# algbio/GraphChainer

Measured on AMD Instinct MI355X. Metric: reads_per_sec, higher is better.
Workload: dtype u64

## Files before the change

graphchainer_amd/csrc/hip/gc_column_asm.hpp:

```cpp
#pragma once

#define GC_CA_NL "\n\t"
#define GC_CA_SELECT \
	"s_and_b32 m0, s90, 6" GC_CA_NL "s_lshr_b64 s[90:91], s[90:91], 2" GC_CA_NL "s_movrels_b64 %[Eq], s[72:73]" GC_CA_NL
#define GC_CA_COLUMN(M0SET, HN, HP, HNMH, FORCE, STORE) \
	GC_CA_SELECT \
	M0SET GC_CA_NL \
	"s_or_b64 %[Xv], %[Eq], s[82:83]" GC_CA_NL \
	HN \
	"s_and_b64 s[84:85], %[Eq], s[80:81]" GC_CA_NL \
	"s_add_u32 s84, s84, s80" GC_CA_NL \
	"s_addc_u32 s85, s85, s81" GC_CA_NL \
	"s_xor_b64 s[84:85], s[84:85], s[80:81]" GC_CA_NL \
	"s_or_b64 s[84:85], s[84:85], %[Eq]" GC_CA_NL           \
	"s_or_b64 %[Eq], s[84:85], s[80:81]" GC_CA_NL \
	"s_orn2_b64 s[86:87], s[82:83], %[Eq]" GC_CA_NL         \
	"s_and_b64 s[88:89], s[80:81], s[84:85]" GC_CA_NL       \
	"v_writelane_b32 %[plus], s87, m0" GC_CA_NL \
	"v_writelane_b32 %[minus], s89, m0" GC_CA_NL \
	"s_lshl_b64 s[84:85], s[86:87], 1" GC_CA_NL \
	HP                                                      \
	"s_lshl_b64 s[88:89], s[88:89], 1" GC_CA_NL \
	HNMH                                                    \
	"s_or_b64 %[Eq], %[Xv], s[84:85]" GC_CA_NL \
	"s_orn2_b64 s[80:81], s[88:89], %[Eq]" GC_CA_NL         \
	"s_and_b64 s[82:83], s[84:85], %[Xv]" GC_CA_NL          \
	FORCE \
	STORE

#define GC_CA_HN "s_bfe_u64 %[hN], %[pHN], m0" GC_CA_NL "s_or_b64 %[Eq], %[Eq], %[hN]" GC_CA_NL
#define GC_CA_HP "s_bfe_u64 %[Eq], %[pHP], m0" GC_CA_NL "s_or_b64 s[84:85], s[84:85], %[Eq]" GC_CA_NL
#define GC_CA_HP_ONE "s_or_b32 s84, s84, 1" GC_CA_NL
#define GC_CA_HNMH "s_or_b64 s[88:89], s[88:89], %[hN]" GC_CA_NL
#define GC_CA_FORCE "s_bfe_u64 %[hN], %[forced], m0" GC_CA_NL "s_andn2_b64 s[80:81], s[80:81], %[hN]" GC_CA_NL "s_or_b64 s[82:83], s[82:83], %[hN]" GC_CA_NL
#define GC_CA_STORE \
	"v_writelane_b32 %[c0], s80, m0" GC_CA_NL "v_writelane_b32 %[c1], s81, m0" GC_CA_NL "v_writelane_b32 %[c2], s82, m0" GC_CA_NL "v_writelane_b32 %[c3], s83, m0" GC_CA_NL
#define GC_CA_NONE ""

#define GC_CA_LOOP(HN, HP, HNMH, FORCE, STORE) \
	"s_lshr_b64 s[90:91], %[w0], 1" GC_CA_NL \
	"s_min_i32 %[endm1], %[nm1], 0x1001f" GC_CA_NL \
	"s_mov_b32 %[pos], 0x10001\n" \
	"1:" GC_CA_NL                                           \
	"s_cmp_ge_i32 %[pos], %[endm1]" GC_CA_NL \
	"s_cbranch_scc1 3f\n" \
	"2:" GC_CA_NL \
	GC_CA_COLUMN("s_mov_b32 m0, %[pos]", HN, HP, HNMH, FORCE, STORE) \
	GC_CA_COLUMN("s_add_i32 m0, %[pos], 1", HN, HP, HNMH, FORCE, STORE) \
	"s_add_i32 %[pos], %[pos], 2" GC_CA_NL \
	"s_cmp_lt_i32 %[pos], %[endm1]" GC_CA_NL \
	"s_cbranch_scc1 2b\n" \
	"3:" GC_CA_NL                                           \
	"s_cmp_gt_i32 %[pos], %[endm1]" GC_CA_NL \
	"s_cbranch_scc1 4f" GC_CA_NL \
	GC_CA_COLUMN("s_mov_b32 m0, %[pos]", HN, HP, HNMH, FORCE, STORE) \
	"s_add_i32 %[pos], %[pos], 1\n" \
	"4:" GC_CA_NL                                           \
	"s_cmp_ge_i32 %[endm1], %[nm1]" GC_CA_NL \
	"s_cbranch_scc1 6f" GC_CA_NL \
	"s_bitcmp1_b32 %[endm1], 5" GC_CA_NL \
	"s_cbranch_scc1 5f" GC_CA_NL \
	"s_lshl_b64 s[90:91], %[w1], 1" GC_CA_NL \
	"s_min_i32 %[endm1], %[nm1], 0x1003e" GC_CA_NL \
	"s_branch 1b\n" \
	"5:" GC_CA_NL \
	"s_lshr_b64 s[90:91], %[w1], 61" GC_CA_NL \
	"s_mov_b32 %[endm1], %[nm1]" GC_CA_NL \
	"s_branch 1b\n" \
	"6:"

#define GC_CA_OUT_COMMON [VP] "+{s[80:81]}"(VP), [VN] "+{s[82:83]}"(VN), [plus] "+v"(plusWord), [minus] "+v"(minusWord), [Eq] "=&s"(Eq), [Xv] "=&s"(Xv), [pos] "=&s"(pos), [endm1] "=&s"(endm1)
#define GC_CA_OUT_STORE , [c0] "+v"(cr[0]), [c1] "+v"(cr[1]), [c2] "+v"(cr[2]), [c3] "+v"(cr[3])
#define GC_CA_IN_COMMON "{s[72:73]}"(eA), "{s[74:75]}"(eC), "{s[76:77]}"(eG), "{s[78:79]}"(eT), [w0] "s"(w0), [w1] "s"(w1), [nm1] "s"(nm1)
#define GC_CA_CLOBBER "s84", "s85", "s86", "s87", "s88", "s89", "s90", "s91", "m0", "scc"

#if defined(__HIP_DEVICE_COMPILE__)
template <int KIND, int MODE>
__device__ __forceinline__ void gcColumnLoopAsm(uint64_t eA, uint64_t eC, uint64_t eG, uint64_t eT, uint64_t& VP, uint64_t& VN, uint64_t prevHP, uint64_t prevHN, uint64_t forced,
	uint64_t w0, uint64_t w1, int nodeLength, uint32_t& plusWord, uint32_t& minusWord, uint32_t* cr)
{
	const uint32_t nm1 = (uint32_t)__builtin_amdgcn_readfirstlane((nodeLength - 1) | (1 << 16));
	uint64_t Eq, Xv, hN;
	uint32_t pos, endm1;
#pragma clang diagnostic push
#pragma clang diagnostic ignored "-Winline-asm"
	if constexpr (KIND == 2 && MODE == 0)
		asm(GC_CA_LOOP(GC_CA_NONE, GC_CA_HP_ONE, GC_CA_NONE, GC_CA_NONE, GC_CA_NONE)
			: GC_CA_OUT_COMMON : GC_CA_IN_COMMON : GC_CA_CLOBBER);
	else if constexpr (KIND == 2)
		asm(GC_CA_LOOP(GC_CA_NONE, GC_CA_HP_ONE, GC_CA_NONE, GC_CA_NONE, GC_CA_STORE)
			: GC_CA_OUT_COMMON GC_CA_OUT_STORE : GC_CA_IN_COMMON : GC_CA_CLOBBER);
	else if constexpr (KIND == 1 && MODE == 0)
		asm(GC_CA_LOOP(GC_CA_HN, GC_CA_HP, GC_CA_HNMH, GC_CA_NONE, GC_CA_NONE)
			: GC_CA_OUT_COMMON, [hN] "=&s"(hN) : GC_CA_IN_COMMON, [pHP] "s"(prevHP), [pHN] "s"(prevHN) : GC_CA_CLOBBER);
	else if constexpr (KIND == 1)
		asm(GC_CA_LOOP(GC_CA_HN, GC_CA_HP, GC_CA_HNMH, GC_CA_NONE, GC_CA_STORE)
			: GC_CA_OUT_COMMON, [hN] "=&s"(hN) GC_CA_OUT_STORE : GC_CA_IN_COMMON, [pHP] "s"(prevHP), [pHN] "s"(prevHN) : GC_CA_CLOBBER);
	else if constexpr (MODE == 0)
		asm(GC_CA_LOOP(GC_CA_HN, GC_CA_HP, GC_CA_HNMH, GC_CA_FORCE, GC_CA_NONE)
			: GC_CA_OUT_COMMON, [hN] "=&s"(hN) : GC_CA_IN_COMMON, [pHP] "s"(prevHP), [pHN] "s"(prevHN), [forced] "s"(forced) : GC_CA_CLOBBER);
	else
		asm(GC_CA_LOOP(GC_CA_HN, GC_CA_HP, GC_CA_HNMH, GC_CA_FORCE, GC_CA_STORE)
			: GC_CA_OUT_COMMON, [hN] "=&s"(hN) GC_CA_OUT_STORE : GC_CA_IN_COMMON, [pHP] "s"(prevHP), [pHN] "s"(prevHN), [forced] "s"(forced) : GC_CA_CLOBBER);
#pragma clang diagnostic pop
}
#endif
```

graphchainer_amd/csrc/hip/gc_device.hpp:

```cpp
#pragma once
#include <hip/hip_runtime.h>
#include <stdint.h>

#ifndef GC_LOOP_TICK
#define GC_LOOP_TICK(i) ((void)0)
#endif

namespace gcdev {

struct NodeRec {
	uint32_t comp;
	uint32_t outOff;
	uint32_t inOff;
	uint32_t meta;
	uint64_t w0, w1;
};
enum : uint32_t { NODEREC_SLOW = 128u };

struct DGraph {
	uint32_t nNodes;
	uint32_t firstAmbiguous;
	const uint8_t*  nodeLength;
	const uint32_t* nodeOffset;
	const int32_t*  nodeIDs;
// ... 247 lines not shown
{
	uint64_t a = 0, c = 0, g = 0, t = 0;
	int n = len - j;
	if (n > 64) n = 64;
	for (int i = 0; i < n; i++) {
		uint32_t m = iupac[(uint8_t)seq[j + i]];
		uint64_t bit = 1ull << i;
		a |= (m & 1) ? bit : 0ull;
		c |= (m & 2) ? bit : 0ull;
		g |= (m & 4) ? bit : 0ull;
		t |= (m & 8) ? bit : 0ull;
	}
	eq.a = a; eq.c = c; eq.g = g; eq.t = t;
}

struct EqSource {
	const uint64_t* masks;
	uint32_t words;
	uint32_t startBit;
	__device__ __forceinline__ void rows(int len, int j, Eq4& eq) const;
};
__device__ inline void eqVectorBits(const EqSource& src, int len, int j, Eq4& eq)
{
	int n = len - j;
	if (n > 64) n = 64;
	uint32_t bit = src.startBit + (uint32_t)j;
	uint32_t w = bit >> 6, sh = bit & 63;
	uint64_t keep = n >= 64 ? ~0ull : ((1ull << n) - 1);
	uint64_t out[4];
	for (int b = 0; b < 4; b++) {
		const uint64_t* v = src.masks + (size_t)b * src.words;
		uint64_t lo = v[w] >> sh;
		uint64_t hi = (sh != 0 && w + 1 < src.words) ? (v[w + 1] << (64 - sh)) : 0ull;
		out[b] = (lo | hi) & keep;
	}
	eq.a = out[0]; eq.c = out[1]; eq.g = out[2]; eq.t = out[3];
}
__device__ __forceinline__ void EqSource::rows(int len, int j, Eq4& eq) const { eqVectorBits(*this, len, j, eq); }

struct NodeSeq { uint64_t w0, w1, w2, w3; bool ambiguous; };
__device__ __forceinline__ NodeSeq loadNodeSeq(const DGraph& g, uint32_t node)
{
	NodeSeq s;
	if (node < g.firstAmbiguous) {
		s.w0 = g.nodeSeq[2 * (size_t)node];
		s.w1 = g.nodeSeq[2 * (size_t)node + 1];
		s.w2 = s.w3 = 0;
		s.ambiguous = false;
	} else {
		const uint64_t* p = g.ambSeq + 4 * (size_t)(node - g.firstAmbiguous);
		s.w0 = p[0]; s.w1 = p[1]; s.w2 = p[2]; s.w3 = p[3];
		s.ambiguous = true;
	}
	return s;
}
__device__ __forceinline__ NodeSeq recNodeSeq(const DGraph& g, uint32_t node, const NodeRec& r)
{
	NodeSeq s;
	if (!(r.meta & NODEREC_SLOW)) {
		s.w0 = r.w0; s.w1 = r.w1;
		s.w2 = s.w3 = 0;
		s.ambiguous = false;
	} else {
		const uint64_t* p = g.ambSeq + 4 * (size_t)(node - g.firstAmbiguous);
		s.w0 = gcK(p); s.w1 = gcK(p + 1); s.w2 = gcK(p + 2); s.w3 = gcK(p + 3);
		s.ambiguous = true;
	}
	return s;
}
__device__ __forceinline__ uint64_t eqOfColumn(const Eq4& eq, const NodeSeq& s, int pos)
{
	if (!s.ambiguous) {
		uint64_t w = pos < 32 ? s.w0 : s.w1;
		uint32_t code = (uint32_t)(w >> ((pos & 31) * 2));
		uint64_t lo = (code & 1) ? eq.c : eq.a;
		uint64_t hi = (code & 1) ? eq.t : eq.g;
		return (code & 2) ? hi : lo;
	}
	uint64_t r = 0;
	r |= ((s.w0 >> pos) & 1) ? eq.a : 0ull;
	r |= ((s.w1 >> pos) & 1) ? eq.c : 0ull;
	r |= ((s.w2 >> pos) & 1) ? eq.g : 0ull;
	r |= ((s.w3 >> pos) & 1) ? eq.t : 0ull;
	return r;
}

__device__ inline int findItem(const uint32_t* itemNodes, const SliceInfo& sl, uint32_t node)
{
	for (uint32_t i = 0; i < sl.count; i++)
		if (itemNodes[sl.first + i] == node) return (int)(sl.first + i);
	return -1;
}

__device__ __forceinline__ int32_t clipXScore(int32_t cells, int32_t scoreHere, double errorCost)
{
#pragma clang fp contract(off)
	const double product = (double)scoreHere * errorCost;
	const double difference = (double)cells - product;
	return (int32_t)difference;
}
__device__ inline int32_t clipMaxXScore(const WS& w, double errorCost, int cells)
{
	const int32_t scoreBeforeStart = wsBefore(w);
	const uint64_t priorityCausedMinima = ~w.VP;
	uint64_t possibleLocalMinima = w.VP & (priorityCausedMinima - w.VP);
	possibleLocalMinima >>= 1;
	possibleLocalMinima |= (1ull << 63) & (priorityCausedMinima | ~(priorityCausedMinima - w.VP)) & ~w.VP;
	int32_t result = INT32_MIN;
	possibleLocalMinima |= 1;
	while (possibleLocalMinima != 0) {
		GC_LOOP_TICK(2);
		const uint64_t currentMinimumMask = possibleLocalMinima ^ (possibleLocalMinima - 1);
		const int cellsHere = popc64(currentMinimumMask);
		if (cellsHere > cells) break;
		const int32_t scoreHere = scoreBeforeStart + popc64(w.VP & currentMinimumMask) - popc64(w.VN & currentMinimumMask);
		const int32_t x = clipXScore(cellsHere, scoreHere, errorCost);
		result = x > result ? x : result;
		possibleLocalMinima &= ~currentMinimumMask;
	}
	return result;
}
struct ClipFind {
	int32_t target;
	int cells;
	bool found; uint32_t column; int row; int32_t value;
};
__device__ inline void clipFindColumn(ClipFind& f, const WS& w, uint32_t column, double errorCost, uint32_t& status)
{
	const int32_t maxScore = clipMaxXScore(w, errorCost, f.cells);
	if (maxScore > f.target) status = EXT_ASSERT;
	if (maxScore != f.target) return;
	for (int off = 63; off >= 0; off--) {
		if (off >= f.cells) continue;
		const int32_t scoreHere = clipXScore(off + 1, wsValue(w, off), errorCost);
		if (scoreHere > f.target) status = EXT_ASSERT;
		if (scoreHere == f.target && (!f.found || off > f.row)) { f.found = true; f.column = column; f.row = off; f.value = wsValue(w, off); }
	}
}

struct TileResult { int32_t minScore; uint32_t minOffset; int32_t flatMin; uint32_t flatOffset; };
template <bool CLIP = false>
__device__ inline TileResult computeTile(const DGraph& g, uint32_t node, WS ws, bool prevExists, int32_t prevStartScore, uint64_t prevHP, uint64_t prevHN,
	const Eq4& eq, NodeItem& out, WCol* columns, int flatRows, uint32_t& status, uint32_t colMask = 63, uint32_t colStride = 1, int lastColumn = 63,
	double errorCost = 0, int32_t* maxX = nullptr, ClipFind* find = nullptr)
{
	int nodeLength = g.nodeLength[node];
	if (lastColumn + 1 < nodeLength) nodeLength = lastColumn + 1;
	NodeSeq seq = loadNodeSeq(g, node);
	TileResult r;
	r.minScore = ws.score;
	r.minOffset = 0;
	if (CLIP && maxX) *maxX = clipMaxXScore(ws, errorCost, 64);
	if (prevExists && wsBefore(ws) > prevStartScore) ws = wsMerge(ws, wsSource(prevStartScore));
	int forceUntil = 0;
	if (prevExists) {
		int32_t scoreBefore = wsBefore(ws);
		int32_t scoreComparison = prevStartScore;
		if (scoreBefore > scoreComparison) status = EXT_ASSERT;
		if (scoreBefore < scoreComparison) {
			for (int fix = 1; fix < 64; fix++) {
				int32_t next = scoreComparison + (int32_t)((prevHP >> fix) & 1) - (int32_t)((prevHN >> fix) & 1);
				uint64_t mask = 1ull << fix;
				if (scoreBefore > next) status = EXT_ASSERT;
				if (scoreBefore < next) { prevHP |= mask; prevHN &= ~mask; forceUntil = fix; }
				if (scoreBefore == next) { prevHP &= ~mask; prevHN &= ~mask; }
				scoreBefore++;
// ... 518 lines not shown
```

graphchainer_amd/csrc/hip/gc_device_wave.hpp:

```cpp
#pragma once
#include "gc_device.hpp"
#include "gc_column_asm.hpp"
#include <type_traits>

namespace gcdev {


#ifndef WAVE_CAP
#define WAVE_CAP 28
#endif

#define WAVE_ENTRY_WORDS 7
#define WAVE_WORDS (3 * WAVE_CAP * WAVE_ENTRY_WORDS)
template <int LANES> struct WaveLdsT { uint32_t w[WAVE_WORDS][LANES]; };
typedef WaveLdsT<64> WaveLds;
static_assert(sizeof(WaveLds) <= 160 * 1024, "WaveLds must fit the CU's LDS");
static_assert(64 * 5 <= WAVE_WORDS, "the 64 backtrace columns (5 words each) alias the lane's table words");

#define WAVE_SPILL 228
#define WAVE_MAX_ENTRIES (WAVE_CAP + WAVE_SPILL)
#define WAVE_SPILL_WORDS (3 * WAVE_SPILL * 4)

typedef __attribute__((address_space(3))) uint32_t lds_u32;

// ... 55 lines not shown
#pragma clang diagnostic push
#pragma clang diagnostic ignored "-Winline-asm"
			asm("s_mov_b32 m0, %7\n\tv_writelane_b32 %0, %8, m0\n\tv_writelane_b32 %1, %9, m0\n\tv_writelane_b32 %2, %10, m0\n\tv_writelane_b32 %3, %11, m0\n\tv_writelane_b32 %4, %12, m0\n\tv_writelane_b32 %5, %13, m0\n\tv_writelane_b32 %6, %14, m0"
				: "+v"(tw[t][0]), "+v"(tw[t][1]), "+v"(tw[t][2]), "+v"(tw[t][3]), "+v"(tw[t][4]), "+v"(tw[t][5]), "+v"(tw[t][6])
				: "s"(es), "s"(v0), "s"(v1), "s"(v2), "s"((uint32_t)a), "s"((uint32_t)(a >> 32)), "s"((uint32_t)b), "s"((uint32_t)(b >> 32)) : "m0");
#pragma clang diagnostic pop
			return;
		}
#endif
		if (REGCOLS) {
			const bool mine = threadIdx.x == e;
			tw[t][0] = mine ? x.w0 : tw[t][0]; tw[t][1] = mine ? x.w1 : tw[t][1]; tw[t][2] = mine ? x.w2 : tw[t][2];
			tw[t][3] = mine ? (uint32_t)x.a : tw[t][3]; tw[t][4] = mine ? (uint32_t)(x.a >> 32) : tw[t][4];
			tw[t][5] = mine ? (uint32_t)x.b : tw[t][5]; tw[t][6] = mine ? (uint32_t)(x.b >> 32) : tw[t][6];
			return;
		}
		if (e < WAVE_CAP) {
			uint32_t base = ldsBase(t, e);
			stL(base, x.w0); stL(base + 1, x.w1); stL(base + 2, x.w2); stL64(base + 3, x.a); stL64(base + 5, x.b);
		} else {
			uint32_t base = spillBase(t, e);
			S(base) = (unsigned long long)x.w0 | ((unsigned long long)x.w1 << 32); S(base + 1) = x.w2; S(base + 2) = x.a; S(base + 3) = x.b;
		}
	}
	__device__ __forceinline__ void rotate() const { for (int k = 0; k < 7; k++) tw[0][k] = tw[1][k]; }
	__device__ __forceinline__ uint32_t word0(uint32_t t, uint32_t e) const { if (REGCOLS) return (uint32_t)GC_READLANE(tw[t][0], e); return e < WAVE_CAP ? ldL(ldsBase(t, e)) : (uint32_t)S(spillBase(t, e)); }
	__device__ __forceinline__ uint32_t word1(uint32_t t, uint32_t e) const { if (REGCOLS) return (uint32_t)GC_READLANE(tw[t][1], e); return e < WAVE_CAP ? ldL(ldsBase(t, e) + 1) : (uint32_t)(S(spillBase(t, e)) >> 32); }
	__device__ __forceinline__ uint32_t word2(uint32_t t, uint32_t e) const { if (REGCOLS) return (uint32_t)GC_READLANE(tw[t][2], e); return e < WAVE_CAP ? ldL(ldsBase(t, e) + 2) : (uint32_t)S(spillBase(t, e) + 1); }
	__device__ __forceinline__ int find(uint32_t t, uint32_t n, uint32_t node) const
	{
		if (REGCOLS) {
			unsigned long long m = __ballot(tw[t][0] == node);
			if (n < 64) m &= (1ull << n) - 1;
			return m ? __ffsll((long long)m) - 1 : -1;
		}
		for (uint32_t i = 0; i < n; i++) if (word0(t, i) == node) return (int)i;
		return -1;
	}
	__device__ __forceinline__ uint32_t pNode(int b, uint32_t e) const { return word0((uint32_t)b, e); }
	__device__ __forceinline__ int32_t pStart(int b, uint32_t e) const { return (int32_t)word1((uint32_t)b, e); }
	__device__ __forceinline__ int32_t pMin(int b, uint32_t e) const { return (int32_t)word2((uint32_t)b, e); }
	__device__ __forceinline__ void pSet(int b, uint32_t e, uint32_t node, int32_t start, int32_t mn, uint64_t hp, uint64_t hn) const { set((uint32_t)b, e, Entry { node, (uint32_t)start, (uint32_t)mn, hp, hn }); }
	__device__ __forceinline__ uint32_t qNode(uint32_t e) const { return word0(2u, e); }
	__device__ __forceinline__ uint32_t qComp(uint32_t e) const { return word1(2u, e); }
	__device__ __forceinline__ WS qWs(uint32_t e) const { Entry x = get(2u, e); return WS { x.a, x.b, (int32_t)x.w2 }; }
	__device__ __forceinline__ void qSet(uint32_t e, uint32_t node, uint32_t comp, const WS& x) const { set(2u, e, Entry { node, comp, (uint32_t)x.score, x.VP, x.VN }); }
	__device__ __forceinline__ void qSetWs(uint32_t e, const WS& x) const { Entry old = get(2u, e); set(2u, e, Entry { old.w0, old.w1, (uint32_t)x.score, x.VP, x.VN }); }
	__device__ __forceinline__ void qMove(uint32_t dst, uint32_t src) const { set(2u, dst, get(2u, src)); }
	__device__ __forceinline__ uint32_t qArgMin(uint32_t n) const
	{
#if defined(__HIP_DEVICE_COMPILE__)
		if (REGCOLS) {
			const uint32_t mine = threadIdx.x < n ? tw[2][1] : 0xffffffffu;
			uint32_t v = mine;
			auto lower = [](uint32_t a, uint32_t b) { return a < b ? a : b; };
			v = lower(v, (uint32_t)__builtin_amdgcn_update_dpp((int)0xffffffffu, (int)v, 0x111, 0xf, 0xf, false));
			v = lower(v, (uint32_t)__builtin_amdgcn_update_dpp((int)0xffffffffu, (int)v, 0x112, 0xf, 0xf, false));
			v = lower(v, (uint32_t)__builtin_amdgcn_update_dpp((int)0xffffffffu, (int)v, 0x114, 0xf, 0xf, false));
			v = lower(v, (uint32_t)__builtin_amdgcn_update_dpp((int)0xffffffffu, (int)v, 0x118, 0xf, 0xf, false));
			v = lower(v, (uint32_t)__builtin_amdgcn_update_dpp((int)0xffffffffu, (int)v, 0x142, 0xa, 0xf, false));
			v = lower(v, (uint32_t)__builtin_amdgcn_update_dpp((int)0xffffffffu, (int)v, 0x143, 0xc, 0xf, false));
			const uint32_t smallest = (uint32_t)GC_READLANE(v, 63);
			const unsigned long long at = __ballot(mine == smallest && threadIdx.x < n);
			return (uint32_t)__ffsll((long long)at) - 1u;
		}
#endif
		uint32_t best = 0;
		uint32_t bestComp = qComp(0);
		for (uint32_t i = 1; i < n; i++) { uint32_t c = qComp(i); if (c < bestComp) { bestComp = c; best = i; } }
		return best;
	}
	mutable uint32_t cr[5];
	mutable uint32_t idCur, idPrev;
	static constexpr bool eqInLanes = REGCOLS;
	mutable uint32_t wm[4] = { 0, 0, 0, 0 };
	mutable bool walkMasks = false;
#if defined(__HIP_DEVICE_COMPILE__)
	__device__ __forceinline__ void setWalkMasks(uint64_t codes0, uint64_t codes1, const Eq4& eq, uint64_t forceEq, uint64_t prevHN) const
	{
		const uint32_t c = threadIdx.x;
		const uint32_t p0 = (uint32_t)__builtin_amdgcn_update_dpp(0, (int)cr[0], 0x138, 0xf, 0xf, false), p1 = (uint32_t)__builtin_amdgcn_update_dpp(0, (int)cr[1], 0x138, 0xf, 0xf, false);
		const uint32_t n0 = (uint32_t)__builtin_amdgcn_update_dpp(0, (int)cr[2], 0x138, 0xf, 0xf, false), n1 = (uint32_t)__builtin_amdgcn_update_dpp(0, (int)cr[3], 0x138, 0xf, 0xf, false);
		const uint64_t pVP = (uint64_t)p0 | ((uint64_t)p1 << 32), pVN = (uint64_t)n0 | ((uint64_t)n1 << 32);
		const uint32_t code = (uint32_t)((c < 32 ? codes0 : codes1) >> ((c & 31u) * 2)) & 3u;
		const uint64_t rawEq = code == 0 ? eq.a : code == 1 ? eq.c : code == 2 ? eq.g : eq.t;
		const uint64_t Eq = (rawEq & forceEq) | ((prevHN >> c) & 1ull);
		const uint64_t Xh = (((Eq & pVP) + pVP) ^ pVP) | Eq;
		const uint64_t Ph = pVN | ~(Xh | pVP), Mh = pVP & Xh;
		const uint64_t flat = ~(Ph | Mh), level = ~(pVP | pVN);
		const uint64_t same = (flat & level) | (Ph & pVN) | (Mh & pVP);
		const uint64_t more = (Ph & level) | (flat & pVP);
		const uint64_t diag = (same & rawEq) | (more & ~rawEq);
		wm[0] = (uint32_t)diag; wm[1] = (uint32_t)(diag >> 32); wm[2] = (uint32_t)Ph; wm[3] = (uint32_t)(Ph >> 32);
		walkMasks = true;
	}
	__device__ __forceinline__ void loadWalkMasks(uint32_t c, uint64_t& up, uint64_t& diag, uint64_t& left) const
	{
		up = (uint64_t)(uint32_t)GC_READLANE(cr[0], c) | ((uint64_t)(uint32_t)GC_READLANE(cr[1], c) << 32);
		diag = (uint64_t)(uint32_t)GC_READLANE(wm[0], c) | ((uint64_t)(uint32_t)GC_READLANE(wm[1], c) << 32);
		left = (uint64_t)(uint32_t)GC_READLANE(wm[2], c) | ((uint64_t)(uint32_t)GC_READLANE(wm[3], c) << 32);
	}
#endif
	__device__ __forceinline__ void colSet(uint32_t c, const WS& x) const
	{
		if (REGCOLS) {
			const bool mine = threadIdx.x == c;
			cr[0] = mine ? (uint32_t)x.VP : cr[0];
			cr[1] = mine ? (uint32_t)(x.VP >> 32) : cr[1];
			cr[2] = mine ? (uint32_t)x.VN : cr[2];
			cr[3] = mine ? (uint32_t)(x.VN >> 32) : cr[3];
			cr[4] = mine ? (uint32_t)x.score : cr[4];
		} else { uint32_t base = c * 5; stL64(base, x.VP); stL64(base + 2, x.VN); stL(base + 4, (uint32_t)x.score); }
	}
	__device__ __forceinline__ WS col(uint32_t c) const
	{
		if (REGCOLS) {
			uint32_t a0 = (uint32_t)GC_READLANE((int)cr[0], (int)c), a1 = (uint32_t)GC_READLANE((int)cr[1], (int)c);
			uint32_t b0 = (uint32_t)GC_READLANE((int)cr[2], (int)c), b1 = (uint32_t)GC_READLANE((int)cr[3], (int)c);
			return WS { (uint64_t)a0 | ((uint64_t)a1 << 32), (uint64_t)b0 | ((uint64_t)b1 << 32), GC_READLANE((int)cr[4], (int)c) };
		}
		uint32_t base = c * 5;
		return WS { ldL64(base), ldL64(base + 2), (int32_t)ldL(base + 4) };
	}
};
typedef LaneLdsT<false> LaneLds;

struct WaveScratch {
	unsigned long long* base;
	uint32_t lane, lanes;
	uint32_t maxSlices, maxItems, maxTrace;
	uint32_t maxCols;
	uint32_t regCap;
	bool allLanes;
	__device__ __forceinline__ bool storer() const { return !allLanes || threadIdx.x == 0; }
	__device__ __forceinline__ unsigned long long& word(uint64_t w) const { return base[w * lanes + lane]; }
	__device__ __forceinline__ uint64_t sliceBase(uint32_t s) const { return (uint64_t)s * 4; }
	__device__ __forceinline__ uint64_t itemBase(uint32_t i) const { return (uint64_t)maxSlices * 4 + (uint64_t)i * 8; }
	__device__ __forceinline__ uint64_t traceBase(uint32_t t, uint32_t which) const { return (uint64_t)maxSlices * 4 + (uint64_t)maxItems * 8 + (uint64_t)which * maxTrace + t; }
	__device__ __forceinline__ uint64_t colBase() const { return (uint64_t)maxSlices * 4 + (uint64_t)maxItems * 8 + 2ull * maxTrace; }
	__device__ __forceinline__ unsigned long long* spillBase() const { return base + ((uint64_t)maxSlices * 4 + (uint64_t)maxItems * 8 + 2ull * maxTrace + 2ull * maxCols) * lanes; }
};
__host__ __device__ inline uint64_t waveScratchWords(uint32_t maxSlices, uint32_t maxItems, uint32_t maxTrace, uint32_t maxCols = 0) { return (uint64_t)maxSlices * 4 + (uint64_t)maxItems * 8 + 2ull * maxTrace + 2ull * maxCols + WAVE_SPILL_WORDS; }

struct WSlice { int32_t minScore; uint32_t minNode, minOffset, first, count; int32_t bandwidth; int32_t j; uint32_t flags; };
__device__ __forceinline__ void setClipScore(WSlice& s, uint32_t node, int32_t x) { s.minNode = node; s.minOffset = (uint32_t)x; }
__device__ __forceinline__ int32_t clipScore(const WSlice& s) { return (int32_t)s.minOffset; }
__device__ __forceinline__ uint32_t clipNode(const WSlice& s) { return s.minNode; }

__device__ __forceinline__ void storeSlice(const WaveScratch& ws, uint32_t s, const WSlice& x)
{
	uint64_t b = ws.sliceBase(s);
	if (!ws.storer()) return;
	ws.word(b) = ((unsigned long long)(uint32_t)x.minScore << 32) | x.minNode;
	ws.word(b + 1) = ((unsigned long long)x.minOffset << 32) | x.first;
	ws.word(b + 2) = ((unsigned long long)x.count << 32) | (uint32_t)x.bandwidth;
	ws.word(b + 3) = ((unsigned long long)(uint32_t)x.j << 32) | x.flags;
}
__device__ __forceinline__ WSlice loadSlice(const WaveScratch& ws, uint32_t s)
{
	uint64_t b = ws.sliceBase(s);
	unsigned long long a = ws.word(b), c = ws.word(b + 1), d = ws.word(b + 2), e = ws.word(b + 3);
	WSlice x;
	x.minScore = (int32_t)(a >> 32); x.minNode = (uint32_t)a;
	x.minOffset = (uint32_t)(c >> 32); x.first = (uint32_t)c;
	x.count = (uint32_t)(d >> 32); x.bandwidth = (int32_t)(uint32_t)d;
	x.j = (int32_t)(e >> 32); x.flags = (uint32_t)e;
	return x;
}
__device__ __forceinline__ void storeItem(const WaveScratch& ws, uint32_t i, const NodeItem& it)
// ... 40 lines not shown
	const int32_t beforeA = wsBefore(a), beforeB = wsBefore(b);
	const int32_t va = beforeA + popc64(a.VP & upTo) - popc64(a.VN & upTo);
	const int32_t vb = beforeB + popc64(b.VP & upTo) - popc64(b.VN & upTo);
	const int32_t m = va < vb ? va : vb;
	const int32_t beforeMin = beforeA < beforeB ? beforeA : beforeB;
	int32_t above = __builtin_amdgcn_update_dpp(0, m, 0x138, 0xf, 0xf, false);
	if (threadIdx.x == 0) above = beforeMin;
	WS res;
	res.VP = __ballot(m == above + 1);
	res.VN = __ballot(m == above - 1);
	res.score = a.score < b.score ? a.score : b.score;
	return res;
}
#endif

struct TilePreamble { uint64_t prevHP, prevHN, forceEq; int forceUntil; };
template <bool ROWS_IN_LANES>
__device__ __forceinline__ int32_t clipMaxXScoreWave(const WS& w, double errorCost)
{
#if defined(__HIP_DEVICE_COMPILE__)
	if (ROWS_IN_LANES) {
		const uint64_t upTo = ~(~1ull << threadIdx.x);
		const int32_t value = wsBefore(w) + popc64(w.VP & upTo) - popc64(w.VN & upTo);
		int32_t x = clipXScore((int32_t)threadIdx.x + 1, value, errorCost);
		auto higher = [](int32_t a, int32_t b) { return a > b ? a : b; };
		x = higher(x, __builtin_amdgcn_update_dpp(INT32_MIN, x, 0x111, 0xf, 0xf, false));
		x = higher(x, __builtin_amdgcn_update_dpp(INT32_MIN, x, 0x112, 0xf, 0xf, false));
		x = higher(x, __builtin_amdgcn_update_dpp(INT32_MIN, x, 0x114, 0xf, 0xf, false));
		x = higher(x, __builtin_amdgcn_update_dpp(INT32_MIN, x, 0x118, 0xf, 0xf, false));
		x = higher(x, __builtin_amdgcn_update_dpp(INT32_MIN, x, 0x142, 0xa, 0xf, false));
		x = higher(x, __builtin_amdgcn_update_dpp(INT32_MIN, x, 0x143, 0xc, 0xf, false));
		return (int32_t)GC_READLANE(x, 63);
	}
#endif
	return clipMaxXScore(w, errorCost, 64);
}
template <int MODE, bool CLIP = false, typename LANE_TABLES>
__device__ __forceinline__ TileResult computeTileW(const DGraph& g, uint32_t node, const NodeRec& rec, WS ws, bool prevExists, int32_t prevStartScore, uint64_t prevHP, uint64_t prevHN,
	const Eq4& eq, NodeItem& out, const LANE_TABLES& tables, int flatRows, uint32_t& status, TilePreamble* preambleOnly = nullptr, double errorCost = 0, int32_t* maxX = nullptr)
{
	constexpr bool COLUMNS = MODE == 1;
	int nodeLength = (int)recLength(rec);
	NodeSeq seq = recNodeSeq(g, node, rec);
	TileResult r;
	r.minScore = ws.score;
	r.minOffset = 0;
	if (CLIP && maxX) *maxX = clipMaxXScoreWave<LANE_TABLES::eqInLanes>(ws, errorCost);
#if defined(__HIP_DEVICE_COMPILE__)
	if (prevExists && wsBefore(ws) > prevStartScore) ws = LANE_TABLES::eqInLanes ? wsMergeWave(ws, wsSource(prevStartScore)) : wsMerge(ws, wsSource(prevStartScore));
#else
	if (prevExists && wsBefore(ws) > prevStartScore) ws = wsMerge(ws, wsSource(prevStartScore));
#endif
	int forceUntil = 0;
	if (prevExists) {
		int32_t scoreBefore = wsBefore(ws);
		int32_t scoreComparison = prevStartScore;
		if (scoreBefore > scoreComparison) status = EXT_ASSERT;
		if (scoreBefore < scoreComparison) {
			for (int fix = 1; fix < 64; fix++) {
				int32_t next = scoreComparison + (int32_t)((prevHP >> fix) & 1) - (int32_t)((prevHN >> fix) & 1);
				uint64_t mask = 1ull << fix;
				if (scoreBefore > next) status = EXT_ASSERT;
				if (scoreBefore < next) { prevHP |= mask; prevHN &= ~mask; forceUntil = fix; }
				if (scoreBefore == next) { prevHP &= ~mask; prevHN &= ~mask; }
				scoreBefore++;
				scoreComparison = next;
				if (scoreBefore >= scoreComparison) break;
			}
		}
	} else {
		forceUntil = nodeLength;
	}
	out.node = node;
	out.sVP = ws.VP; out.sVN = ws.VN; out.sScore = ws.score;
	uint64_t flatMask = flatRows > 0 ? ~(~0ull << flatRows) : 0;
	r.flatMin = INT32_MAX;
	r.flatOffset = 0;
	if (flatRows > 0) r.flatMin = ws.score - popc64(ws.VP & ~flatMask) + popc64(ws.VN & ~flatMask);
	if (COLUMNS) tables.colSet(0, ws);
	uint64_t forceEq = prevExists ? ~0ull : ~1ull;
	if (preambleOnly) { preambleOnly->prevHP = prevHP; preambleOnly->prevHN = prevHN; preambleOnly->forceEq = forceEq; preambleOnly->forceUntil = forceUntil; return r; }
#if defined(__HIP_DEVICE_COMPILE__)
	if (!CLIP && LANE_TABLES::eqInLanes && !seq.ambiguous && flatRows <= 0) {
		const uint64_t eA = gcUniform64(eq.a & forceEq), eC = gcUniform64(eq.c & forceEq), eG = gcUniform64(eq.g & forceEq), eT = gcUniform64(eq.t & forceEq);
		const uint64_t forced = gcUniform64(forceUntil >= 63 ? ~0ull : ((2ull << forceUntil) - 1));
		prevHP = gcUniform64(prevHP); prevHN = gcUniform64(prevHN);
		uint64_t VP = ws.VP, VN = ws.VN;
		uint32_t plusWord = 0, minusWord = 0;
		auto columnLoop = [&, &plusWord = plusWord, &minusWord = minusWord, &tables = tables](auto kindTag) __attribute__((always_inline)) {
			gcColumnLoopAsm<decltype(kindTag)::value, MODE>(eA, eC, eG, eT, VP, VN, prevHP, prevHN, forced, gcUniform64(seq.w0), gcUniform64(seq.w1), nodeLength, plusWord, minusWord, tables.cr);
		};
		if (!prevExists) columnLoop(std::integral_constant<int, 2>());
		else if (forceUntil == 0) columnLoop(std::integral_constant<int, 1>());
		else columnLoop(std::integral_constant<int, 0>());
		const uint64_t HP = __ballot((int32_t)plusWord < 0), HN = __ballot((int32_t)minusWord < 0);
		out.HP = HP; out.HN = HN;
		out.eVP = VP; out.eVN = VN; out.eScore = ws.score + popc64(HP) - popc64(HN);
		if (nodeLength > 1) {
			int32_t run = (int32_t)(plusWord >> 31) - (int32_t)(minusWord >> 31);
			run += __builtin_amdgcn_update_dpp(0, run, 0x111, 0xf, 0xf, false);
			run += __builtin_amdgcn_update_dpp(0, run, 0x112, 0xf, 0xf, false);
			run += __builtin_amdgcn_update_dpp(0, run, 0x114, 0xf, 0xf, false);
			run += __builtin_amdgcn_update_dpp(0, run, 0x118, 0xf, 0xf, false);
			run += __builtin_amdgcn_update_dpp(0, run, 0x142, 0xa, 0xf, false);
			run += __builtin_amdgcn_update_dpp(0, run, 0x143, 0xc, 0xf, false);
			const int32_t columnScore = ws.score + run;
			if (COLUMNS) {
				if (threadIdx.x >= 1 && threadIdx.x < (uint32_t)nodeLength) tables.cr[4] = (uint32_t)columnScore;
			} else {
				uint32_t key = threadIdx.x == 0 ? ((uint32_t)r.minScore << 6) : threadIdx.x < (uint32_t)nodeLength ? (((uint32_t)columnScore << 6) | threadIdx.x) : 0xffffffffu;
				auto lower = [](uint32_t a, uint32_t b) { return a < b ? a : b; };
				key = lower(key, (uint32_t)__builtin_amdgcn_update_dpp(-1, (int)key, 0x111, 0xf, 0xf, false));
				key = lower(key, (uint32_t)__builtin_amdgcn_update_dpp(-1, (int)key, 0x112, 0xf, 0xf, false));
				key = lower(key, (uint32_t)__builtin_amdgcn_update_dpp(-1, (int)key, 0x114, 0xf, 0xf, false));
				key = lower(key, (uint32_t)__builtin_amdgcn_update_dpp(-1, (int)key, 0x118, 0xf, 0xf, false));
				key = lower(key, (uint32_t)__builtin_amdgcn_update_dpp(-1, (int)key, 0x142, 0xa, 0xf, false));
				key = lower(key, (uint32_t)__builtin_amdgcn_update_dpp(-1, (int)key, 0x143, 0xc, 0xf, false));
				const uint32_t minKey = (uint32_t)GC_READLANE(key, 63);
				r.minScore = (int32_t)(minKey >> 6);
				r.minOffset = minKey & 63u;
			}
		}
		if (COLUMNS) tables.setWalkMasks(seq.w0, seq.w1, eq, forceEq, prevHN);
		return r;
	}
	if (COLUMNS && LANE_TABLES::eqInLanes) tables.walkMasks = false;
#endif
	uint64_t HP = 0, HN = 0;
	for (int pos = 1; pos < nodeLength; pos++) {
		uint64_t Eq;
		Eq = eqOfColumn(eq, seq, pos);
		Eq &= forceEq;
		uint64_t hp, hn;
		ws = myersStep(Eq, ws, (prevHP >> pos) & 1, (prevHN >> pos) & 1, hp, hn);
		{ const uint64_t f = (uint64_t)((uint32_t)(pos - forceUntil - 1) >> 31); ws.VP &= ~f; ws.VN |= f; }
		if (ws.score < r.minScore) { r.minScore = ws.score; r.minOffset = (uint32_t)pos; }
		if (flatRows > 0) {
			int32_t f = ws.score - popc64(ws.VP & ~flatMask) + popc64(ws.VN & ~flatMask);
			if (f < r.flatMin) { r.flatMin = f; r.flatOffset = (uint32_t)pos; }
		}
		if (MODE != 0) tables.colSet((uint32_t)pos, ws);
		if (CLIP && maxX) { const int32_t x = clipMaxXScoreWave<LANE_TABLES::eqInLanes>(ws, errorCost); *maxX = x > *maxX ? x : *maxX; }
		HP |= hp << pos;
		HN |= hn << pos;
	}
	out.HP = HP; out.HN = HN;
	out.eVP = ws.VP; out.eVN = ws.VN; out.eScore = ws.score;
	return r;
}


template <bool REGCOLS, bool BAND = false, bool CLIP = false>
__device__ __forceinline__ uint32_t extendSeedWave(const DGraph& g, const CorrectnessTables& ct, const EqSource& eqSrc, int bandwidthCfg, lds_u32* lds, const WaveScratch& wsx,
	int len, uint32_t startNode, uint32_t startOffset, uint32_t which, uint32_t& nTrace, int32_t& score, ExtCounters& cnt, int rampBandwidth = 0, uint32_t maxCells = ~0u, bool forceGlobal = false,
	double errorCost = 0, int32_t xDrop = 0)
{
	static_assert(BAND || !CLIP, "CLIP is instantiated with BAND");
	const LaneLdsT<REGCOLS> L { lds, wsx.lane, wsx.lanes, wsx.spillBase(), {}, wsx.regCap < 64 ? wsx.regCap : 64u, { 0, 0, 0, 0, 0 }, 0, 0 };
	uint32_t status = EXT_OK;
	nTrace = 0;
	score = 0;
	cnt.extensions++;
	cnt.flattenTie = 0;
	int numSlices = (len + 63) / 64;
	if ((uint32_t)numSlices + 1 > wsx.maxSlices) return EXT_OVERFLOW;
	int buf = 0;
	uint32_t nPrev = 1;
	{
		int nl = (int)gcNodeLength(g, startNode);
		NodeItem it;
		it.node = startNode;
		it.sVP = it.sVN = it.eVP = it.eVN = 0;
		it.sScore = (int32_t)startOffset;
// ... 665 lines not shown
```

Baseline: 79200.

## Precompute per-column Eq masks in lanes and read them via readlane in asm loop

```diff
diff --git a/graphchainer_amd/csrc/hip/gc_column_asm.hpp b/graphchainer_amd/csrc/hip/gc_column_asm.hpp
--- a/graphchainer_amd/csrc/hip/gc_column_asm.hpp
+++ b/graphchainer_amd/csrc/hip/gc_column_asm.hpp
@@ -1,20 +1,19 @@
 #pragma once
 
 #define GC_CA_NL "\n\t"
-#define GC_CA_SELECT \
-	"s_and_b32 m0, s90, 6" GC_CA_NL "s_lshr_b64 s[90:91], s[90:91], 2" GC_CA_NL "s_movrels_b64 %[Eq], s[72:73]" GC_CA_NL
-#define GC_CA_COLUMN(M0SET, HN, HP, HNMH, FORCE, STORE) \
-	GC_CA_SELECT \
+#define GC_CA_COLUMN(EQ, N0, N1, M0SET, HN, HP, HNMH, FORCE, STORE) \
 	M0SET GC_CA_NL \
-	"s_or_b64 %[Xv], %[Eq], s[82:83]" GC_CA_NL \
+	"s_or_b64 %[Xv], " EQ ", s[82:83]" GC_CA_NL \
+	"v_readlane_b32 " N0 ", %[e0], m0" GC_CA_NL \
+	"v_readlane_b32 " N1 ", %[e1], m0" GC_CA_NL \
 	HN \
-	"s_and_b64 s[84:85], %[Eq], s[80:81]" GC_CA_NL \
+	"s_and_b64 s[84:85], " EQ ", s[80:81]" GC_CA_NL \
 	"s_add_u32 s84, s84, s80" GC_CA_NL \
 	"s_addc_u32 s85, s85, s81" GC_CA_NL \
 	"s_xor_b64 s[84:85], s[84:85], s[80:81]" GC_CA_NL \
-	"s_or_b64 s[84:85], s[84:85], %[Eq]" GC_CA_NL           \
-	"s_or_b64 %[Eq], s[84:85], s[80:81]" GC_CA_NL \
-	"s_orn2_b64 s[86:87], s[82:83], %[Eq]" GC_CA_NL         \
+	"s_or_b64 s[84:85], s[84:85], " EQ GC_CA_NL             \
+	"s_or_b64 s[76:77], s[84:85], s[80:81]" GC_CA_NL \
+	"s_orn2_b64 s[86:87], s[82:83], s[76:77]" GC_CA_NL      \
 	"s_and_b64 s[88:89], s[80:81], s[84:85]" GC_CA_NL       \
 	"v_writelane_b32 %[plus], s87, m0" GC_CA_NL \
 	"v_writelane_b32 %[minus], s89, m0" GC_CA_NL \
@@ -22,14 +21,16 @@
 	HP                                                      \
 	"s_lshl_b64 s[88:89], s[88:89], 1" GC_CA_NL \
 	HNMH                                                    \
-	"s_or_b64 %[Eq], %[Xv], s[84:85]" GC_CA_NL \
-	"s_orn2_b64 s[80:81], s[88:89], %[Eq]" GC_CA_NL         \
+	"s_or_b64 s[76:77], %[Xv], s[84:85]" GC_CA_NL \
+	"s_orn2_b64 s[80:81], s[88:89], s[76:77]" GC_CA_NL      \
 	"s_and_b64 s[82:83], s[84:85], %[Xv]" GC_CA_NL          \
 	FORCE \
 	STORE
+#define GC_CA_COLUMN_A(M0SET, HN, HP, HNMH, FORCE, STORE) GC_CA_COLUMN("s[72:73]", "s74", "s75", M0SET, HN, HP, HNMH, FORCE, STORE)
+#define GC_CA_COLUMN_B(M0SET, HN, HP, HNMH, FORCE, STORE) GC_CA_COLUMN("s[74:75]", "s72", "s73", M0SET, HN, HP, HNMH, FORCE, STORE)
 
-#define GC_CA_HN "s_bfe_u64 %[hN], %[pHN], m0" GC_CA_NL "s_or_b64 %[Eq], %[Eq], %[hN]" GC_CA_NL
-#define GC_CA_HP "s_bfe_u64 %[Eq], %[pHP], m0" GC_CA_NL "s_or_b64 s[84:85], s[84:85], %[Eq]" GC_CA_NL
+#define GC_CA_HN "s_bfe_u64 %[hN], %[pHN], m0" GC_CA_NL
+#define GC_CA_HP "s_bfe_u64 s[76:77], %[pHP], m0" GC_CA_NL "s_or_b64 s[84:85], s[84:85], s[76:77]" GC_CA_NL
 #define GC_CA_HP_ONE "s_or_b32 s84, s84, 1" GC_CA_NL
 #define GC_CA_HNMH "s_or_b64 s[88:89], s[88:89], %[hN]" GC_CA_NL
 #define GC_CA_FORCE "s_bfe_u64 %[hN], %[forced], m0" GC_CA_NL "s_andn2_b64 s[80:81], s[80:81], %[hN]" GC_CA_NL "s_or_b64 s[82:83], s[82:83], %[hN]" GC_CA_NL
@@ -38,50 +39,36 @@
 #define GC_CA_NONE ""
 
 #define GC_CA_LOOP(HN, HP, HNMH, FORCE, STORE) \
-	"s_lshr_b64 s[90:91], %[w0], 1" GC_CA_NL \
-	"s_min_i32 %[endm1], %[nm1], 0x1001f" GC_CA_NL \
-	"s_mov_b32 %[pos], 0x10001\n" \
-	"1:" GC_CA_NL                                           \
-	"s_cmp_ge_i32 %[pos], %[endm1]" GC_CA_NL \
-	"s_cbranch_scc1 3f\n" \
+	"s_mov_b32 %[pos], 0x10001" GC_CA_NL \
+	"s_cmp_ge_i32 %[pos], %[nm1]" GC_CA_NL \
+	"v_readlane_b32 s72, %[e0], 0" GC_CA_NL \
+	"v_readlane_b32 s73, %[e1], 0" GC_CA_NL \
+	"s_cbranch_scc1 3f\n"                                   \
 	"2:" GC_CA_NL \
-	GC_CA_COLUMN("s_mov_b32 m0, %[pos]", HN, HP, HNMH, FORCE, STORE) \
-	GC_CA_COLUMN("s_add_i32 m0, %[pos], 1", HN, HP, HNMH, FORCE, STORE) \
+	GC_CA_COLUMN_A("s_mov_b32 m0, %[pos]", HN, HP, HNMH, FORCE, STORE) \
+	GC_CA_COLUMN_B("s_add_i32 m0, %[pos], 1", HN, HP, HNMH, FORCE, STORE) \
 	"s_add_i32 %[pos], %[pos], 2" GC_CA_NL \
-	"s_cmp_lt_i32 %[pos], %[endm1]" GC_CA_NL \
+	"s_cmp_lt_i32 %[pos], %[nm1]" GC_CA_NL \
 	"s_cbranch_scc1 2b\n" \
 	"3:" GC_CA_NL                                           \
-	"s_cmp_gt_i32 %[pos], %[endm1]" GC_CA_NL \
+	"s_cmp_gt_i32 %[pos], %[nm1]" GC_CA_NL \
 	"s_cbranch_scc1 4f" GC_CA_NL \
-	GC_CA_COLUMN("s_mov_b32 m0, %[pos]", HN, HP, HNMH, FORCE, STORE) \
-	"s_add_i32 %[pos], %[pos], 1\n" \
-	"4:" GC_CA_NL                                           \
-	"s_cmp_ge_i32 %[endm1], %[nm1]" GC_CA_NL \
-	"s_cbranch_scc1 6f" GC_CA_NL \
-	"s_bitcmp1_b32 %[endm1], 5" GC_CA_NL \
-	"s_cbranch_scc1 5f" GC_CA_NL \
-	"s_lshl_b64 s[90:91], %[w1], 1" GC_CA_NL \
-	"s_min_i32 %[endm1], %[nm1], 0x1003e" GC_CA_NL \
-	"s_branch 1b\n" \
-	"5:" GC_CA_NL \
-	"s_lshr_b64 s[90:91], %[w1], 61" GC_CA_NL \
-	"s_mov_b32 %[endm1], %[nm1]" GC_CA_NL \
-	"s_branch 1b\n" \
-	"6:"
+	GC_CA_COLUMN_A("s_mov_b32 m0, %[pos]", HN, HP, HNMH, FORCE, STORE) \
+	"\n4:"
 
-#define GC_CA_OUT_COMMON [VP] "+{s[80:81]}"(VP), [VN] "+{s[82:83]}"(VN), [plus] "+v"(plusWord), [minus] "+v"(minusWord), [Eq] "=&s"(Eq), [Xv] "=&s"(Xv), [pos] "=&s"(pos), [endm1] "=&s"(endm1)
+#define GC_CA_OUT_COMMON [VP] "+{s[80:81]}"(VP), [VN] "+{s[82:83]}"(VN), [plus] "+v"(plusWord), [minus] "+v"(minusWord), [Xv] "=&s"(Xv), [pos] "=&s"(pos)
 #define GC_CA_OUT_STORE , [c0] "+v"(cr[0]), [c1] "+v"(cr[1]), [c2] "+v"(cr[2]), [c3] "+v"(cr[3])
-#define GC_CA_IN_COMMON "{s[72:73]}"(eA), "{s[74:75]}"(eC), "{s[76:77]}"(eG), "{s[78:79]}"(eT), [w0] "s"(w0), [w1] "s"(w1), [nm1] "s"(nm1)
-#define GC_CA_CLOBBER "s84", "s85", "s86", "s87", "s88", "s89", "s90", "s91", "m0", "scc"
+#define GC_CA_IN_COMMON [e0] "v"(eqLo), [e1] "v"(eqHi), [nm1] "s"(nm1)
+#define GC_CA_CLOBBER "s72", "s73", "s74", "s75", "s76", "s77", "s84", "s85", "s86", "s87", "s88", "s89", "m0", "scc"
 
 #if defined(__HIP_DEVICE_COMPILE__)
 template <int KIND, int MODE>
-__device__ __forceinline__ void gcColumnLoopAsm(uint64_t eA, uint64_t eC, uint64_t eG, uint64_t eT, uint64_t& VP, uint64_t& VN, uint64_t prevHP, uint64_t prevHN, uint64_t forced,
-	uint64_t w0, uint64_t w1, int nodeLength, uint32_t& plusWord, uint32_t& minusWord, uint32_t* cr)
+__device__ __forceinline__ void gcColumnLoopAsm(uint32_t eqLo, uint32_t eqHi, uint64_t& VP, uint64_t& VN, uint64_t prevHP, uint64_t prevHN, uint64_t forced,
+	int nodeLength, uint32_t& plusWord, uint32_t& minusWord, uint32_t* cr)
 {
 	const uint32_t nm1 = (uint32_t)__builtin_amdgcn_readfirstlane((nodeLength - 1) | (1 << 16));
-	uint64_t Eq, Xv, hN;
-	uint32_t pos, endm1;
+	uint64_t Xv, hN;
+	uint32_t pos;
 #pragma clang diagnostic push
 #pragma clang diagnostic ignored "-Winline-asm"
 	if constexpr (KIND == 2 && MODE == 0)
diff --git a/graphchainer_amd/csrc/hip/gc_device.hpp b/graphchainer_amd/csrc/hip/gc_device.hpp
--- a/graphchainer_amd/csrc/hip/gc_device.hpp
+++ b/graphchainer_amd/csrc/hip/gc_device.hpp
@@ -353,6 +353,23 @@
 	r |= ((s.w1 >> pos) & 1) ? eq.c : 0ull;
 	r |= ((s.w2 >> pos) & 1) ? eq.g : 0ull;
 	r |= ((s.w3 >> pos) & 1) ? eq.t : 0ull;
+	return r;
+}
+
+struct LaneInputs { uint64_t raw, masked, eq, hp, hn, forced; };
+__host__ __device__ inline LaneInputs laneInputs(uint32_t c, uint64_t w0, uint64_t w1, const Eq4& eq, uint64_t forceEq, uint64_t prevHP, uint64_t prevHN, int forceUntil)
+{
+	c &= 63u;
+	const uint32_t code = (uint32_t)((c < 32 ? w0 : w1) >> ((c & 31u) * 2));
+	const uint64_t lo = (code & 1) ? eq.c : eq.a;
+	const uint64_t hi = (code & 1) ? eq.t : eq.g;
+	LaneInputs r;
+	r.raw = (code & 2) ? hi : lo;
+	r.masked = r.raw & forceEq;
+	r.hp = (prevHP >> c) & 1ull;
+	r.hn = (prevHN >> c) & 1ull;
+	r.eq = r.masked | r.hn;
+	r.forced = (int)c <= forceUntil ? 1ull : 0ull;
 	return r;
 }
 
diff --git a/graphchainer_amd/csrc/hip/gc_device_wave.hpp b/graphchainer_amd/csrc/hip/gc_device_wave.hpp
--- a/graphchainer_amd/csrc/hip/gc_device_wave.hpp
+++ b/graphchainer_amd/csrc/hip/gc_device_wave.hpp
@@ -161,9 +161,8 @@
 		const uint32_t p0 = (uint32_t)__builtin_amdgcn_update_dpp(0, (int)cr[0], 0x138, 0xf, 0xf, false), p1 = (uint32_t)__builtin_amdgcn_update_dpp(0, (int)cr[1], 0x138, 0xf, 0xf, false);
 		const uint32_t n0 = (uint32_t)__builtin_amdgcn_update_dpp(0, (int)cr[2], 0x138, 0xf, 0xf, false), n1 = (uint32_t)__builtin_amdgcn_update_dpp(0, (int)cr[3], 0x138, 0xf, 0xf, false);
 		const uint64_t pVP = (uint64_t)p0 | ((uint64_t)p1 << 32), pVN = (uint64_t)n0 | ((uint64_t)n1 << 32);
-		const uint32_t code = (uint32_t)((c < 32 ? codes0 : codes1) >> ((c & 31u) * 2)) & 3u;
-		const uint64_t rawEq = code == 0 ? eq.a : code == 1 ? eq.c : code == 2 ? eq.g : eq.t;
-		const uint64_t Eq = (rawEq & forceEq) | ((prevHN >> c) & 1ull);
+		const LaneInputs in = laneInputs(c, codes0, codes1, eq, forceEq, 0, prevHN, 0);
+		const uint64_t rawEq = in.raw, Eq = in.eq;
 		const uint64_t Xh = (((Eq & pVP) + pVP) ^ pVP) | Eq;
 		const uint64_t Ph = pVN | ~(Xh | pVP), Mh = pVP & Xh;
 		const uint64_t flat = ~(Ph | Mh), level = ~(pVP | pVN);
@@ -370,13 +369,16 @@
 	if (preambleOnly) { preambleOnly->prevHP = prevHP; preambleOnly->prevHN = prevHN; preambleOnly->forceEq = forceEq; preambleOnly->forceUntil = forceUntil; return r; }
 #if defined(__HIP_DEVICE_COMPILE__)
 	if (!CLIP && LANE_TABLES::eqInLanes && !seq.ambiguous && flatRows <= 0) {
-		const uint64_t eA = gcUniform64(eq.a & forceEq), eC = gcUniform64(eq.c & forceEq), eG = gcUniform64(eq.g & forceEq), eT = gcUniform64(eq.t & forceEq);
+		{
+			const LaneInputs in = laneInputs(threadIdx.x + 1, seq.w0, seq.w1, eq, forceEq, 0, prevExists ? prevHN : 0ull, 0);
+			tables.wm[0] = (uint32_t)in.eq; tables.wm[1] = (uint32_t)(in.eq >> 32);
+		}
 		const uint64_t forced = gcUniform64(forceUntil >= 63 ? ~0ull : ((2ull << forceUntil) - 1));
 		prevHP = gcUniform64(prevHP); prevHN = gcUniform64(prevHN);
 		uint64_t VP = ws.VP, VN = ws.VN;
 		uint32_t plusWord = 0, minusWord = 0;
 		auto columnLoop = [&, &plusWord = plusWord, &minusWord = minusWord, &tables = tables](auto kindTag) __attribute__((always_inline)) {
-			gcColumnLoopAsm<decltype(kindTag)::value, MODE>(eA, eC, eG, eT, VP, VN, prevHP, prevHN, forced, gcUniform64(seq.w0), gcUniform64(seq.w1), nodeLength, plusWord, minusWord, tables.cr);
+			gcColumnLoopAsm<decltype(kindTag)::value, MODE>(tables.wm[0], tables.wm[1], VP, VN, prevHP, prevHN, forced, nodeLength, plusWord, minusWord, tables.cr);
 		};
 		if (!prevExists) columnLoop(std::integral_constant<int, 2>());
 		else if (forceUntil == 0) columnLoop(std::integral_constant<int, 1>());
```

New measurement: 81940, median of 4. 1.03x the previous value.
